# tudelft-iv/CCVPE

Hardware: AMD Instinct MI355X
Metric: image-pairs/sec (higher is better)
Workload: dtype f32

## Files before the change

ccvpe_amd/_lib.py:

```python
import ctypes
import os
import subprocess

import torch

_HERE = os.path.dirname(os.path.abspath(__file__))
LIB_PATH = os.environ.get("CCVPE_LIB") or os.path.join(_HERE, "libccvpe_hip.so")
CSRC_DIR = os.path.join(_HERE, "csrc")

c_float_p = ctypes.c_void_p
c_int = ctypes.c_int
c_float = ctypes.c_float
c_void_p = ctypes.c_void_p


class ConvDesc(ctypes.Structure):
    _fields_ = [
        ("src0", c_void_p), ("src1", c_void_p), ("gate", c_void_p), ("w", c_void_p),
        ("scale", c_void_p), ("shift", c_void_p), ("residual", c_void_p), ("dst", c_void_p),
        ("c0", c_int), ("ld0", c_int), ("c1", c_int), ("ld1", c_int),
        ("batch", c_int), ("in_h", c_int), ("in_w", c_int),
        ("kh", c_int), ("kw", c_int), ("stride", c_int), ("pad", c_int),
        ("n", c_int), ("kpad", c_int), ("ldd", c_int), ("ldres", c_int),
        ("act", c_int), ("out_mode", c_int),
# ... 6 lines not shown
        ("c0", c_int), ("ld0", c_int), ("c1", c_int), ("ld1", c_int),
        ("batch", c_int), ("h1", c_int), ("w1", c_int),
        ("n", c_int), ("kpad", c_int), ("ldd", c_int), ("act", c_int),
    ]


class TailDesc(ctypes.Structure):
    _fields_ = [
        ("x", c_void_p), ("w", c_void_p), ("shift9", c_void_p), ("w2", c_void_p), ("b2", c_void_p), ("out", c_void_p),
        ("batch", c_int), ("h1", c_int), ("w1", c_int),
        ("c0", c_int), ("ld0", c_int), ("kpad", c_int),
        ("cout", c_int), ("normalize", c_int), ("split", c_int), ("softmax_partial", c_void_p),
    ]


PROTOTYPES = {
    "ccvpe_last_error": (ctypes.c_char_p, []),
    "ccvpe_abi_version": (c_int, []),
    "ccvpe_multi_copy_f32": (c_int, [ctypes.POINTER(c_void_p), ctypes.POINTER(c_void_p), ctypes.POINTER(c_int), c_int, c_void_p]),
    "ccvpe_gather_repack_f32": (c_int, [c_void_p, c_void_p, c_void_p, c_void_p, c_void_p, c_int, c_void_p]),
    "ccvpe_gather_repack_chunk": (c_int, []),
    "ccvpe_ctx_create": (c_int, [c_void_p, ctypes.c_longlong, c_void_p, c_void_p, ctypes.POINTER(c_void_p)]),
    "ccvpe_ctx_destroy": (c_int, [c_void_p]),
    "ccvpe_ctx_info": (c_int, [c_void_p] + [ctypes.POINTER(ctypes.c_longlong)] * 4 + [ctypes.POINTER(c_int)] * 2),
    "ccvpe_ctx_output": (c_int, [c_void_p, c_int, ctypes.POINTER(c_void_p), ctypes.POINTER(ctypes.c_longlong),
                                  ctypes.POINTER(c_int), ctypes.POINTER(ctypes.c_longlong), ctypes.POINTER(ctypes.c_longlong)]),
    "ccvpe_forward": (c_int, [c_void_p, c_void_p, c_void_p, ctypes.POINTER(c_void_p), c_void_p]),
    "ccvpe_tail512_partials": (c_int, [ctypes.POINTER(TailDesc), c_int]),
    "ccvpe_softmax_apply_f32": (c_int, [c_void_p, c_void_p, c_int, c_void_p, c_int, c_int, c_void_p]),
    "ccvpe_tail512_f32": (c_int, [ctypes.POINTER(TailDesc), c_void_p]),
    "ccvpe_tail512_bf16": (c_int, [ctypes.POINTER(TailDesc), c_void_p]),
    "ccvpe_conv_igemm_f32": (c_int, [ctypes.POINTER(ConvDesc), c_void_p]),
    "ccvpe_conv_igemm_splitk_floats": (c_int, [ctypes.POINTER(ConvDesc), c_int]),
    "ccvpe_conv_igemm_route": (c_int, [ctypes.POINTER(ConvDesc), c_int, c_int]),
    "ccvpe_set_narrow_kernels": (c_int, [c_int]),
    "ccvpe_set_pw_ring_kernels": (c_int, [c_int]),
    "ccvpe_set_mbconv_plane_kernels": (c_int, [c_int]),
    "ccvpe_mbconv_front_route": (c_int, [c_int] * 8),
    "ccvpe_mbconv_band_plan": (c_int, [c_int] * 7),
    "ccvpe_conv3x3_variant": (c_int, [ctypes.POINTER(ConvDesc), c_int]),
    "ccvpe_set_match_mfma": (c_int, [c_int]),
    "ccvpe_set_pwn_kernels": (c_int, [c_int]),
    "ccvpe_conv3x3_wino_ok": (c_int, [ctypes.POINTER(ConvDesc)]),
    "ccvpe_conv3x3_wino_f32": (c_int, [ctypes.POINTER(ConvDesc), c_void_p]),
    "ccvpe_conv3x3_match1_ok": (c_int, [ctypes.POINTER(ConvDesc), c_int, c_int]),
    "ccvpe_conv3x3_match1_bf16": (c_int, [ctypes.POINTER(ConvDesc), c_int, c_void_p, c_int, c_int, c_int, c_int, c_int, c_void_p, c_void_p]),
    "ccvpe_conv_igemm_splitk_f32": (c_int, [ctypes.POINTER(ConvDesc), c_void_p, c_void_p]),
    "ccvpe_conv_igemm_splitk_bf16": (c_int, [ctypes.POINTER(ConvDesc), c_int, c_void_p, c_void_p]),
    "ccvpe_upconv3x3_f32": (c_int, [ctypes.POINTER(UpconvDesc), c_void_p]),
    "ccvpe_upconv3x3_bf16": (c_int, [ctypes.POINTER(UpconvDesc), c_void_p]),
    "ccvpe_upconv3x3_route": (c_int, [ctypes.POINTER(UpconvDesc), c_int]),
    "ccvpe_upconv3x3_s3_ok": (c_int, [ctypes.POINTER(UpconvDesc)]),
    "ccvpe_upconv3x3_s3_f32": (c_int, [ctypes.POINTER(UpconvDesc), c_void_p]),
    "ccvpe_stem_conv_f32": (c_int, [c_void_p] * 5 + [c_int] * 4 + [c_void_p]),
    "ccvpe_dwconv_nblk": (c_int, [c_int] * 4),
    "ccvpe_dwconv_f32": (c_int, [c_void_p] * 6 + [c_int] * 7 + [c_void_p]),
    "ccvpe_mbconv_front_nblk": (c_int, [c_int] * 6),
    "ccvpe_stem_dw_nblk": (c_int, [c_int] * 3),
    "ccvpe_stem_dw_f32": (c_int, [c_void_p] * 9 + [c_int] * 4 + [c_void_p]),
    "ccvpe_stem_dw_bf16": (c_int, [c_void_p] * 9 + [c_int] * 4 + [c_void_p]),
    "ccvpe_mbconv_front_f32": (c_int, [c_void_p, c_void_p, c_int] + [c_void_p] * 7 + [c_int] * 8 + [c_void_p]),
    "ccvpe_se_gate_f32": (c_int, [c_void_p, c_int, c_float] + [c_void_p] * 5 + [c_int] * 3 + [c_void_p]),
    "ccvpe_ground_descriptor_f32": (c_int, [c_void_p, c_int, c_void_p, c_void_p, ctypes.POINTER(c_int),
                                            c_void_p, c_int, c_int, c_int, c_void_p]),
    "ccvpe_match_level_f32": (c_int, [c_void_p, c_int, c_void_p, c_int, c_int, ctypes.POINTER(c_int),
                                      c_int, c_int, c_int, c_int, c_int, c_void_p, c_void_p, c_int, c_int,
                                      c_int, c_int, c_void_p]),
    "ccvpe_head_conv3x3_f32": (c_int, [c_void_p] * 4 + [c_int] * 5 + [c_void_p]),
    "ccvpe_cast_bf16_f32": (c_int, [c_void_p, c_void_p, ctypes.c_long, c_void_p]),
    "ccvpe_softmax_rows_f32": (c_int, [c_void_p, c_void_p, c_int, c_int, c_void_p]),
    "ccvpe_eval_postprocess_f32": (c_int, [c_void_p, c_void_p, c_void_p, c_int, c_int, c_int, c_void_p]),
    "ccvpe_infonce_scratch_floats": (c_int, [c_int, c_int]),
    "ccvpe_infonce_loss_f32": (c_int, [c_void_p, c_void_p, c_float, c_void_p, c_void_p, c_void_p, c_int, c_int, c_void_p]),
    "ccvpe_cross_entropy_loss_f32": (c_int, [c_void_p] * 4 + [c_int, c_int, c_void_p]),
    "ccvpe_orientation_loss_f32": (c_int, [c_void_p] * 5 + [c_int, c_int, c_void_p]),
    "ccvpe_stem_conv_raw_f32": (c_int, [c_void_p] * 3 + [c_int] * 4 + [c_void_p]),
    "ccvpe_dwconv_raw_f32": (c_int, [c_void_p] * 3 + [c_int] * 7 + [c_void_p]),
    "ccvpe_bn_stats_nblk": (c_int, [c_int]),
    "ccvpe_bn_stats_f32": (c_int, [c_void_p, c_int, c_int] + [c_void_p] * 4 + [c_float, c_void_p, c_void_p]),
    "ccvpe_bn_act_nblk": (c_int, [c_int]),
    "ccvpe_bn_act_f32": (c_int, [c_void_p] * 5 + [c_float, c_int] + [c_void_p] * 4 + [c_int] * 3 + [c_void_p]),
    "ccvpe_conv_wgrad_tile": (c_int, [c_int, c_int]),
    "ccvpe_conv_wgrad_scratch_floats": (c_int, [c_int] * 9),
    "ccvpe_conv_wgrad_f32": (c_int, [c_void_p, c_int, c_int, c_void_p, c_int, c_int, c_void_p, c_int, c_void_p,
                                     c_void_p] + [c_int] * 8 + [c_void_p]),
    "ccvpe_conv_wgrad_gated_f32": (c_int, [c_void_p, c_int, c_int, c_void_p, c_void_p, c_int, c_void_p, c_void_p, c_int, c_int, c_int,
                                           c_int, c_void_p]),
    "ccvpe_conv_wgrad_bias_f32": (c_int, [c_void_p, c_int, c_int, c_void_p, c_int, c_int, c_void_p, c_int, c_void_p,
                                          c_void_p, c_void_p] + [c_int] * 8 + [c_void_p]),
    "ccvpe_colsum_f32": (c_int, [c_void_p, c_int, c_int, c_int, c_void_p, c_void_p, c_void_p]),
    "ccvpe_bn_bwd_nblk": (c_int, [c_int]),
    "ccvpe_bn_act_bwd_f32": (c_int, [c_void_p] * 9 + [c_float, c_int] + [c_void_p] * 4 + [c_int] * 3 + [c_void_p]),
    "ccvpe_se_bn_bwd_reduce_f32": (c_int, [c_void_p] * 6 + [c_float, c_int, c_void_p, c_void_p, c_int, c_int, c_int, c_void_p]),
    "ccvpe_se_bn_bwd_apply_f32": (c_int, [c_void_p] * 8 + [c_float, c_int, c_void_p, c_void_p, c_void_p, c_void_p, c_int, c_int, c_int,
                                          c_void_p]),
    "ccvpe_se_dgate_f32": (c_int, [c_void_p] * 6 + [c_float, c_int, c_void_p] + [c_int] * 3 + [c_void_p]),
    "ccvpe_se_bwd_f32": (c_int, [c_void_p, c_int, c_float, c_void_p, c_int] + [c_void_p] * 10 + [c_int] * 3 + [c_void_p]),
    "ccvpe_dwconv_dgrad_f32": (c_int, [c_void_p] * 3 + [c_int] * 7 + [c_void_p]),
    "ccvpe_dwconv_wgrad_nblk": (c_int, [c_int] * 4),
    "ccvpe_dwconv_wgrad_f32": (c_int, [c_void_p] * 4 + [c_int] * 7 + [c_void_p]),
    "ccvpe_relu_bwd_f32": (c_int, [c_void_p] * 3 + [c_int, c_void_p]),
    "ccvpe_gate_mul_f32": (c_int, [c_void_p] * 3 + [c_int] * 3 + [c_void_p]),
    "ccvpe_softmax_bwd_f32": (c_int, [c_void_p] * 4 + [c_int, c_int, c_void_p]),
    "ccvpe_l2norm2_bwd_f32": (c_int, [c_void_p] * 3 + [c_int, c_int, c_void_p]),
    "ccvpe_head_conv3x3_bwd_f32": (c_int, [c_void_p] * 7 + [c_int] * 5 + [c_void_p]),
    "ccvpe_ground_descriptor_bwd_f32": (c_int, [c_void_p, c_int, c_void_p, ctypes.POINTER(c_int)] + [c_void_p] * 4 +
# ... 16 lines not shown
    "ccvpe_adam_step_f32": (c_int, [c_void_p, c_void_p, c_void_p, c_void_p, c_int, c_float, c_void_p]),
    "ccvpe_preprocess_u8_f32": (c_int, [c_void_p, c_int, c_int, c_void_p, c_void_p, c_int, c_void_p, c_void_p, c_int, c_void_p,
                                        c_void_p, c_int, c_int, c_int, c_int, ctypes.POINTER(c_float), ctypes.POINTER(c_float),
                                        c_void_p]),
    "ccvpe_conv_igemm_bf16": (c_int, [ctypes.POINTER(ConvDesc), c_int, c_void_p]),
    "ccvpe_stem_conv_bf16": (c_int, [c_void_p] * 5 + [c_int] * 4 + [c_void_p]),
    "ccvpe_dwconv_bf16": (c_int, [c_void_p] * 6 + [c_int] * 7 + [c_void_p]),
    "ccvpe_mbconv_front_bf16": (c_int, [c_void_p, c_void_p, c_int] + [c_void_p] * 7 + [c_int] * 8 + [c_void_p]),
    "ccvpe_match_level_bf16": (c_int, [c_void_p, c_int, c_void_p, c_int, c_int, ctypes.POINTER(c_int),
                                       c_int, c_int, c_int, c_int, c_int, c_void_p, c_void_p, c_int, c_int,
                                       c_int, c_int, c_void_p]),
    "ccvpe_head_conv3x3_bf16": (c_int, [c_void_p] * 4 + [c_int] * 5 + [c_void_p]),
}

_lib = None
weights_epoch = 0


def build(verbose=False):
    cmd = ["make", "-C", CSRC_DIR, "-j8"]
    res = subprocess.run(cmd, capture_output=True, text=True)
    if verbose or res.returncode != 0:
        print(res.stdout)
        print(res.stderr)
    if res.returncode != 0:
        raise RuntimeError("building libccvpe_hip.so failed (see output above)")
    return LIB_PATH


def load():
    global _lib
    if _lib is not None:
        return _lib
    if not os.path.isfile(LIB_PATH):
        raise RuntimeError(
            "libccvpe_hip.so not found at %s — run `python -c 'import __graft_entry__ as g; g.build()'` "
            "(or `make -C ccvpe_amd/csrc`).  ccvpe_amd has no CPU fallback." % LIB_PATH)
    lib = ctypes.CDLL(LIB_PATH)
    lax = bool(os.environ.get("CCVPE_LIB")) and os.environ.get("CCVPE_LIB_ALLOW_MISSING") == "1"
    for name, (res, args) in PROTOTYPES.items():
        if lax and not hasattr(lib, name):
            continue
        fn = getattr(lib, name)
        fn.restype = res
        fn.argtypes = args
    if os.environ.get("CCVPE_NARROW") == "0" and hasattr(lib, "ccvpe_set_narrow_kernels"):
        lib.ccvpe_set_narrow_kernels(0)
    if os.environ.get("CCVPE_PW_RING") == "0" and hasattr(lib, "ccvpe_set_pw_ring_kernels"):
        lib.ccvpe_set_pw_ring_kernels(0)
    if os.environ.get("CCVPE_MATCH_MFMA") == "0" and hasattr(lib, "ccvpe_set_match_mfma"):
        lib.ccvpe_set_match_mfma(0)
    if os.environ.get("CCVPE_PWN") == "0" and hasattr(lib, "ccvpe_set_pwn_kernels"):
        lib.ccvpe_set_pwn_kernels(0)
    if os.environ.get("CCVPE_MBPLANE") is not None and hasattr(lib, "ccvpe_set_mbconv_plane_kernels"):
        lib.ccvpe_set_mbconv_plane_kernels(int(os.environ["CCVPE_MBPLANE"]))
    _lib = lib
    return lib


class CcvpeError(RuntimeError):
    pass


def check(status, what):
    if status != 0:
        msg = load().ccvpe_last_error()
        raise CcvpeError("%s failed (%d): %s" % (what, status, msg.decode() if msg else "?"))
```

ccvpe_amd/csrc/conv_common.h:

```cpp
#pragma once
#include "common.h"
#include <cstdlib>
#include <type_traits>

namespace ccvpe {

typedef float f32x4 __attribute__((ext_vector_type(4)));
typedef __bf16 bf16_t;
typedef __bf16 bf16x8 __attribute__((ext_vector_type(8)));
typedef __bf16 bf16x4 __attribute__((ext_vector_type(4)));

template <typename T> struct ElemTraits;
template <> struct ElemTraits<float> { static constexpr int E = 4; };
template <> struct ElemTraits<bf16_t> { static constexpr int E = 8; };

template <typename T>
__device__ __forceinline__ f32x4 mfma_stage(f32x4 wfrag, f32x4 afrag, f32x4 acc);
template <>
__device__ __forceinline__ f32x4 mfma_stage<float>(f32x4 wfrag, f32x4 afrag, f32x4 acc) {
#pragma unroll
  for (int kk = 0; kk < 4; ++kk) acc = __builtin_amdgcn_mfma_f32_16x16x4f32(wfrag[kk], afrag[kk], acc, 0, 0, 0);
  return acc;
}
template <>
// ... 131 lines not shown
        else reinterpret_cast<bf16_t*>(p.dst)[obase + r] = (bf16_t)t;
      }
  }
}

#define CCVPE_ACT_DISPATCH(act, body)                                            \
  do {                                                                           \
    if ((act) == CCVPE_ACT_SWISH) body(std::integral_constant<int, CCVPE_ACT_SWISH>{});      \
    else if ((act) == CCVPE_ACT_RELU) body(std::integral_constant<int, CCVPE_ACT_RELU>{});   \
    else if ((act) == CCVPE_ACT_RELU_MASK) body(std::integral_constant<int, CCVPE_ACT_RELU_MASK>{}); \
    else body(std::integral_constant<int, CCVPE_ACT_NONE>{});                    \
  } while (0)

__device__ __forceinline__ int w_swz(int r) { return (0x1320 >> (((r >> 2) & 3) * 4)) & 3; }

struct TileCfg { int mt, nt, wn; };
static const TileCfg kCfgs[] = {
    {4, 5, 2}, {4, 4, 2}, {4, 3, 2}, {4, 2, 2}, {4, 1, 2},
    {4, 5, 1}, {4, 3, 1}, {4, 1, 1},
    {2, 7, 1},
};

static int pick_cfg(int npad16) {
  int best = 0;
  long best_cost = -1;
  for (int i = 0; i < (int)(sizeof(kCfgs) / sizeof(kCfgs[0])); ++i) {
    const int bn = 16 * kCfgs[i].nt * kCfgs[i].wn;
    const int tiles = (npad16 + bn - 1) / bn;
    const long cost = (long)tiles * bn * 1000 + (1000 - bn);
    if (best_cost < 0 || cost < best_cost) { best_cost = cost; best = i; }
  }
  return best;
}


template <typename T> int pw_dispatch(const IgemmParams& p, int mt, int nt, int wn, hipStream_t stream);
template <typename T> int conv3x3_dispatch(const IgemmParams& p, int batch, int mt, int nt, int wn, hipStream_t stream);
template <typename T> int conv3x3_variant_query(const IgemmParams& p, int batch, int mt, int nt, int wn);
extern bool g_use_pw2;
template <typename T> bool pw2_supported(const IgemmParams& p, int mt, int nt, int wn);
template <typename T> int pw2_dispatch(const IgemmParams& p, int mt, int nt, int wn, hipStream_t stream);
int num_cus();
extern bool g_use_narrow;
int c3n_supported(const IgemmParams& p, int batch);
int c3n_dispatch(const IgemmParams& p, int batch, hipStream_t stream);
int c3n_match_supported(const IgemmParams& p, int batch, int L);
int c3n_match_dispatch(const IgemmParams& p, int batch, const float* g, int ldg, int L, int off, float* scores, hipStream_t stream);
extern bool g_use_pwn;
bool pwn_supported(const IgemmParams& p, int batch, int esz);
int pwn_dispatch(const IgemmParams& p, int batch, int esz, hipStream_t stream);
int up2_supported(int c0, int c1, int n, int kpad, int h1, int w1, int batch);
int up2_dispatch(const void* src0, const void* src1, const void* w, const float* shift9, void* dst, int c0, int ld0, int c1, int ld1,
                 int h1, int w1, int n, int kpad, int ldd, int act, int batch, hipStream_t stream);

}
```

ccvpe_amd/csrc/upconv_s3.hip:

```cpp
#include "conv_common.h"

namespace ccvpe {

struct UpS3Params {
  const float* src0;
  const float* src1;
  const void* w;
  const float* shift9;
  float* dst;
  int c0, ld0, c1, ld1;
  int H1, W1, batch;
  int N, Npad;
  int nb0, nb1, nst;
  int ldd, act;
  int tiles_n, tiles_total;
};

template <int MT, int NT, int WN, bool PAIR>
struct UpS3Geom {
  static constexpr int WM = 4 / WN;
  static constexpr int BM = 16 * MT * WM;
  static constexpr int BN = 16 * NT * WN;
  static constexpr int TH = BM / 16;
  static constexpr int HR = TH + 2, HCP = PAIR ? 26 : 18;
// ... 284 lines not shown
}

template <int MT, int NT, int WN, bool PAIR>
static int launch_s3(UpS3Params p, hipStream_t stream) {
  using G = UpS3Geom<MT, NT, WN, PAIR>;
  static_assert(G::LDS_BYTES <= 80 * 1024, "upconv_s3_kernel: two workgroups per CU");
  p.tiles_n = (p.Npad + G::BN - 1) / G::BN;
  const long tiles_m = PAIR ? (p.batch + 1) / 2 : (long)((p.W1 + 15) / 16) * ((p.H1 + G::TH - 1) / G::TH) * p.batch;
  const long total = tiles_m * p.tiles_n * 4;
  if (total > 0x7fffffffL) return fail(CCVPE_EINVAL, "upconv_s3: grid too large");
  p.tiles_total = (int)total;
  static bool attr_set = false;
  if (!attr_set) {
    hipError_t e = hipFuncSetAttribute((const void*)upconv_s3_kernel<MT, NT, WN, PAIR>, hipFuncAttributeMaxDynamicSharedMemorySize, G::LDS_BYTES);
    if (e != hipSuccess) return fail(CCVPE_ELAUNCH, "upconv_s3_kernel: set smem attr: %s", hipGetErrorString(e));
    attr_set = true;
  }
  hipLaunchKernelGGL((upconv_s3_kernel<MT, NT, WN, PAIR>), dim3(p.tiles_total), dim3(256), G::LDS_BYTES, stream, p);
  return check_launch("upconv_s3_kernel");
}

static bool s3_tile(int mt, int nt, int wn) {
  return mt == 4 && ((wn == 2 && (nt == 5 || nt == 4 || nt == 2 || nt == 1)) || (wn == 1 && (nt == 5 || nt == 3)));
}

static const char* s3_refusal(const ccvpe_upconv_desc* d) {
  if (!d) return "null desc";
  if (d->c0 <= 0 || d->c0 % 8 || d->c1 <= 0 || d->c1 % 8) return "c0 / c1 must be positive multiples of 8 (a layer without a skip is not implemented)";
  if (d->batch <= 0 || d->h1 <= 0 || d->w1 <= 0 || d->n <= 0) return "bad shape";
  if (d->ld0 < d->c0 || d->ld0 % 4 || d->ld1 < d->c1 || d->ld1 % 4 || d->ldd < d->n || d->ldd % 4) return "bad strides";
  const int nst = 4 * ((d->c0 + 15) / 16) + 9 * ((d->c1 + 15) / 16);
  if (d->kpad != nst * 48) return "kpad is not that of the three-plane pack (models._pack_upconv_s3)";
  const bool pair = d->w1 == 8 && d->h1 == 8;
  if (d->w1 < 16 && !pair) return "low-res images narrower than 16 pixels (other than 8 x 8)";
  const int npad = (d->n + 15) / 16 * 16;
  const TileCfg c = kCfgs[pick_cfg(npad)];
  if (!s3_tile(c.mt, c.nt, c.wn)) return "no tile for this n";
  if (pair && !(c.nt == 5 && c.wn == 2)) return "8 x 8 images need the 160-column tile";
  const double m = (double)d->batch * d->h1 * d->w1;
  if (m * d->ld0 * 4.0 >= 4294967296.0 || 4.0 * m * d->ld1 * 4.0 >= 4294967296.0 || 4.0 * m >= 2147483648.0) return "tensor too large";
  return nullptr;
}

}

using namespace ccvpe;

extern "C" int ccvpe_upconv3x3_s3_ok(const ccvpe_upconv_desc* d) {
  if (s3_refusal(d)) return 0;
  const long m = (long)d->batch * d->h1 * d->w1;
  return m >= 4096 ? 2 : 1;
}

extern "C" int ccvpe_upconv3x3_s3_f32(const ccvpe_upconv_desc* d, void* stream) {
  if (const char* why = s3_refusal(d)) return fail(CCVPE_EINVAL, "upconv3x3_s3: %s", why);
  if (!d->src0 || !d->src1 || !d->w || !d->shift9 || !d->dst) return fail(CCVPE_EINVAL, "upconv3x3_s3: null pointer");
  if (!aligned16(d->src0) || !aligned16(d->src1) || !aligned16(d->w) || !aligned16(d->dst))
    return fail(CCVPE_EINVAL, "upconv3x3_s3: pointers must be 16-byte aligned");
  UpS3Params p;
  p.src0 = reinterpret_cast<const float*>(d->src0); p.src1 = reinterpret_cast<const float*>(d->src1);
  p.w = d->w; p.shift9 = d->shift9; p.dst = reinterpret_cast<float*>(d->dst);
  p.c0 = d->c0; p.ld0 = d->ld0; p.c1 = d->c1; p.ld1 = d->ld1;
  p.H1 = d->h1; p.W1 = d->w1; p.batch = d->batch;
  p.N = d->n; p.Npad = (d->n + 15) / 16 * 16;
  p.nb0 = (d->c0 + 15) / 16; p.nb1 = (d->c1 + 15) / 16; p.nst = 4 * p.nb0 + 9 * p.nb1;
  p.ldd = d->ldd; p.act = d->act;
  p.tiles_n = p.tiles_total = 0;
  hipStream_t st = (hipStream_t)stream;
  const TileCfg c = kCfgs[pick_cfg(p.Npad)];
  if (d->w1 == 8 && d->h1 == 8) return launch_s3<4, 5, 2, true>(p, st);
#define CCVPE_CASE(MT_, NT_, WN_) \
  if (c.mt == MT_ && c.nt == NT_ && c.wn == WN_) return launch_s3<MT_, NT_, WN_, false>(p, st);
  CCVPE_CASE(4, 5, 2) CCVPE_CASE(4, 4, 2) CCVPE_CASE(4, 2, 2) CCVPE_CASE(4, 1, 2) CCVPE_CASE(4, 5, 1) CCVPE_CASE(4, 3, 1)
#undef CCVPE_CASE
  return fail(CCVPE_EINVAL, "upconv3x3_s3: no tile config");
}
```

ccvpe_amd/ops.py:

```python
import ctypes

import torch

from . import _lib
from ._lib import ConvDesc, check

ACT_NONE, ACT_RELU, ACT_SWISH, ACT_RELU_MASK = 0, 1, 2, 3
SPLIT_K_CALLS = 0
SPLIT_K = __import__("os").environ.get("CCVPE_SPLIT_K", "1") == "1"
OUT_NHWC, OUT_DECONV2X = 0, 1

_recorder = None


def set_recorder(rec):
    global _recorder
    _recorder = rec


class LaunchRecorder(object):

    def __init__(self):
        self.items = []

# ... 230 lines not shown
    return dst


def upconv3x3(src0, c0, w_packed, shift9, n, *, batch, h1, w1, src1=None, c1=0, act=ACT_NONE, algo_flops=None, route_only=False):
    lib = _lib.load()
    dt = _act_dtype(src0)
    for t, nm in ((src0, "src0"), (src1, "src1"), (w_packed, "w")):
        _chk(t, nm, dt)
    _chk(shift9, "shift9")
    dst = _empty((batch, 2 * h1, 2 * w1, n), device=src0.device, dtype=dt)
    d = _lib.UpconvDesc()
    d.src0, d.src1, d.w, d.shift9, d.dst = _ptr(src0), _ptr(src1), _ptr(w_packed), _ptr(shift9), _ptr(dst)
    d.c0, d.ld0, d.c1, d.ld1 = c0, src0.shape[-1], c1, (src1.shape[-1] if src1 is not None else 0)
    d.batch, d.h1, d.w1 = batch, h1, w1
    d.n, d.kpad, d.ldd, d.act = n, w_packed.shape[-1], n, act
    if route_only:
        return upconv_route(d, dt != torch.float32)
    rec = _recorder
    ev0 = rec.begin() if rec is not None else None
    fn = lib.ccvpe_upconv3x3_f32 if dt == torch.float32 else lib.ccvpe_upconv3x3_bf16
    check(fn(ctypes.byref(d), _stream()), "ccvpe_upconv3x3")
    if rec is not None:
        m = batch * h1 * w1 * 4
        k_eff = 4 * c0 + 9 * c1
        flops = algo_flops if algo_flops is not None else 2.0 * m * n * k_eff
        esz = 4.0 if dt == torch.float32 else 2.0
        nbytes = esz * (batch * h1 * w1 * c0 + m * c1 + m * n + 4 * n * k_eff)
        name = upconv_route_name(d, dt != torch.float32)
        rec.end(name, "up3x3 M%d N%d Keff%d" % (m, n, k_eff), flops, nbytes, ev0)
    return dst


def _s3_desc(src0, c0, w3_packed, shift9, n, batch, h1, w1, src1, c1, act, dst, ldd, ld0, ld1):
    d = _lib.UpconvDesc()
    d.src0, d.src1, d.w, d.shift9 = _ptr(src0), _ptr(src1), _ptr(w3_packed), _ptr(shift9)
    d.dst = _ptr(dst) if dst is not None else None
    d.c0, d.ld0, d.c1, d.ld1 = c0, ld0, c1, ld1
    d.batch, d.h1, d.w1 = batch, h1, w1
    d.n, d.kpad, d.ldd, d.act = n, w3_packed.shape[1] * w3_packed.shape[3], ldd, act
    return d


def upconv3x3_s3_ok(src0, c0, w3_packed, n, *, batch, h1, w1, src1=None, c1=0, ldd=None, ld0=None, ld1=None):
    if w3_packed is None or src0.dtype != torch.float32 or (src1 is not None and src1.dtype != torch.float32):
        return 0
    if w3_packed.dtype != torch.bfloat16 or w3_packed.dim() != 4:
        return 0
    ld0 = ld0 if ld0 is not None else src0.shape[-1]
    ld1 = ld1 if ld1 is not None else (src1.shape[-1] if src1 is not None else 0)
    d = _s3_desc(src0, c0, w3_packed, None, n, batch, h1, w1, src1, c1, ACT_NONE, None, ldd if ldd is not None else n, ld0, ld1)
    return int(_lib.load().ccvpe_upconv3x3_s3_ok(ctypes.byref(d)))


def upconv3x3_s3(src0, c0, w3_packed, shift9, n, *, batch, h1, w1, src1=None, c1=0, act=ACT_NONE, dst=None, ldd=None, ld0=None,
                 ld1=None):
    lib = _lib.load()
    for t, nm in ((src0, "src0"), (src1, "src1"), (shift9, "shift9"), (dst, "dst")):
        _chk(t, nm)
    _chk(w3_packed, "w", torch.bfloat16)
    ld0 = ld0 if ld0 is not None else src0.shape[-1]
    ld1 = ld1 if ld1 is not None else (src1.shape[-1] if src1 is not None else 0)
    if dst is None:
        ldd = ldd if ldd is not None else n
        dst = _empty((batch, 2 * h1, 2 * w1, ldd), device=src0.device)
    elif ldd is None:
        ldd = dst.shape[-1]
    d = _s3_desc(src0, c0, w3_packed, shift9, n, batch, h1, w1, src1, c1, act, dst, ldd, ld0, ld1)
    rec = _recorder
    ev0 = rec.begin() if rec is not None else None
    check(lib.ccvpe_upconv3x3_s3_f32(ctypes.byref(d), _stream()), "ccvpe_upconv3x3_s3_f32")
    if rec is not None:
        m = batch * h1 * w1 * 4
        k_eff = 4 * c0 + 9 * c1
        flops = 2.0 * m * n * k_eff
        nbytes = 4.0 * (batch * h1 * w1 * c0 + m * c1 + m * n + 4 * n * k_eff)
        tile = igemm_tile(n).split("<")[1]
        name = "upconv_s3_kernel<%s%s" % (tile[:-1], ",pair>" if (h1 == 8 and w1 == 8) else ">")
        rec.end(name, "up3x3 M%d N%d Keff%d" % (m, n, k_eff), flops, nbytes, ev0)
    return dst


def tail512(x, c0, w_packed, shift9, w2, b2, cout, normalize, *, batch, h1, w1, split=False, want_softmax=False):
    lib = _lib.load()
    dt = _act_dtype(x)
    _chk(x, "x", dt)
    _chk(w_packed, "w", dt)
    for t, nm in ((shift9, "shift9"), (w2, "w2"), (b2, "b2")):
        _chk(t, nm)
    if tuple(w2.shape) != (cout, 3, 3, 16) or tuple(shift9.shape) != (9, 16) or w_packed.shape[0] != 4 or w_packed.shape[1] != 16:
        raise ValueError("tail512: w [4,16,kpad], shift9 [9,16], w2 [cout,3,3,16] expected")
    out = _empty((batch, cout, 2 * h1, 2 * w1), device=x.device, dtype=torch.float32)
    d = _lib.TailDesc()
    d.x, d.w, d.shift9, d.w2, d.b2, d.out = _ptr(x), _ptr(w_packed), _ptr(shift9), _ptr(w2), _ptr(b2), _ptr(out)
    d.batch, d.h1, d.w1 = batch, h1, w1
    d.c0, d.ld0, d.kpad = c0, x.shape[-1], w_packed.shape[-1]
    d.cout, d.normalize, d.split = cout, int(bool(normalize)), int(bool(split))
    smx = None
    if want_softmax:
        npart = lib.ccvpe_tail512_partials(ctypes.byref(d), int(dt != torch.float32))
        if npart <= 0:
            check(int(npart) if npart < 0 else -1, "ccvpe_tail512_partials")
        smx = _empty((batch, npart, 2), device=x.device, dtype=torch.float32)
        d.softmax_partial = _ptr(smx)
    rec = _recorder
    ev0 = rec.begin() if rec is not None else None
    fn = lib.ccvpe_tail512_f32 if dt == torch.float32 else lib.ccvpe_tail512_bf16
    check(fn(ctypes.byref(d), _stream()), "ccvpe_tail512")
    if rec is not None:
        m = batch * h1 * w1 * 4
        esz = 4.0 if dt == torch.float32 else 2.0
        rec.end("tail512_kernel<%s,%d>" % (("f32" if not split else "f32 as bf16 hi+lo") if dt == torch.float32 else "bf16", cout), "tail M%d Keff%d" % (m, 4 * c0),
                2.0 * m * 16 * (4 * c0 + 9 * cout), esz * batch * h1 * w1 * c0 + 4.0 * m * cout, ev0)
    return (out, smx) if want_softmax else out


def softmax_apply(logits, partials):
    lib = _lib.load()
    _chk(logits, "logits")
    _chk(partials, "partials")
    rows, n = logits.shape
    out = _empty(logits.shape, device=logits.device, dtype=logits.dtype)
    check(lib.ccvpe_softmax_apply_f32(_ptr(logits), _ptr(partials), partials.shape[1], _ptr(out), rows, n, _stream()),
          "ccvpe_softmax_apply_f32")
    return out


def tail512_ok(h1, w1, n_a):
    return n_a == 16 and h1 % 16 == 0 and w1 % 16 == 0


# ... 333 lines not shown
```

include/ccvpe_hip.h:

```cpp
#ifndef CCVPE_HIP_H
#define CCVPE_HIP_H

#ifdef __cplusplus
extern "C" {
#endif

#define CCVPE_OK 0
#define CCVPE_EINVAL (-1)
#define CCVPE_ELAUNCH (-2)

#define CCVPE_ACT_NONE 0
#define CCVPE_ACT_RELU 1
#define CCVPE_ACT_SWISH 2
#define CCVPE_ACT_RELU_MASK 3

#define CCVPE_OUT_NHWC 0
#define CCVPE_OUT_DECONV2X 1

#define CCVPE_MAX_SHIFTS 48

const char* ccvpe_last_error(void);
int ccvpe_abi_version(void);

typedef struct ccvpe_conv_desc {
// ... 9 lines not shown
  int batch, in_h, in_w;
  int kh, kw, stride, pad;
  int n;
  int kpad;
  int ldd, ldres;
  int act;
  int out_mode;
} ccvpe_conv_desc;

int ccvpe_conv_igemm_f32(const ccvpe_conv_desc* desc, void* stream);

int ccvpe_conv_igemm_splitk_floats(const ccvpe_conv_desc* desc, int is_bf16);
#define CCVPE_ROUTE_IGEMM 0
#define CCVPE_ROUTE_PW_GEMM 1
#define CCVPE_ROUTE_CONV3X3 2
#define CCVPE_ROUTE_C3N 3
#define CCVPE_ROUTE_PW_RING 4
#define CCVPE_ROUTE_PWN 5
int ccvpe_conv_igemm_route(const ccvpe_conv_desc* desc, int is_bf16, int out_f32);
int ccvpe_conv3x3_variant(const ccvpe_conv_desc* desc, int is_bf16);
int ccvpe_set_narrow_kernels(int on);
int ccvpe_set_pw_ring_kernels(int on);
int ccvpe_set_pwn_kernels(int on);
int ccvpe_set_mbconv_plane_kernels(int mode);
int ccvpe_conv3x3_wino_ok(const ccvpe_conv_desc* desc);
int ccvpe_conv3x3_wino_f32(const ccvpe_conv_desc* desc, void* stream);
int ccvpe_conv3x3_match1_ok(const ccvpe_conv_desc* desc, int out_f32, int L);
int ccvpe_conv3x3_match1_bf16(const ccvpe_conv_desc* desc, int out_f32, const float* g, int ldg, int L, int shift, int stride,
                              int window_offset, float* scores, void* stream);
int ccvpe_conv_igemm_splitk_f32(const ccvpe_conv_desc* desc, float* scratch, void* stream);

typedef struct ccvpe_upconv_desc {
  const void* src0;
  const void* src1;
  const void* w;
  const float* shift9;
  void* dst;
  int c0, ld0, c1, ld1;
  int batch, h1, w1;
  int n, kpad, ldd;
  int act;
} ccvpe_upconv_desc;

int ccvpe_upconv3x3_f32(const ccvpe_upconv_desc* desc, void* stream);
int ccvpe_upconv3x3_bf16(const ccvpe_upconv_desc* desc, void* stream);
#define CCVPE_UPROUTE_GATHER 0
#define CCVPE_UPROUTE_HALO 1
#define CCVPE_UPROUTE_DMA 2
#define CCVPE_UPROUTE_DMA_PAIR 3
#define CCVPE_UPROUTE_UP2 4
int ccvpe_upconv3x3_route(const ccvpe_upconv_desc* desc, int is_bf16);
int ccvpe_upconv3x3_s3_ok(const ccvpe_upconv_desc* desc);
int ccvpe_upconv3x3_s3_f32(const ccvpe_upconv_desc* desc, void* stream);

typedef struct ccvpe_tail_desc {
  const void* x;
  const void* w;
  const float* shift9;
  const float* w2;
  const float* b2;
  float* out;
  int batch, h1, w1;
  int c0, ld0, kpad;
  int cout, normalize, split;
  float* softmax_partial;
} ccvpe_tail_desc;

int ccvpe_tail512_f32(const ccvpe_tail_desc* desc, void* stream);
int ccvpe_tail512_bf16(const ccvpe_tail_desc* desc, void* stream);
int ccvpe_tail512_partials(const ccvpe_tail_desc* desc, int is_bf16);
int ccvpe_softmax_apply_f32(const float* logits, const float* partials, int n_partials, float* out, int rows, int n,
                            void* stream);

typedef struct ccvpe_ctx ccvpe_ctx;
int ccvpe_ctx_create(const void* plan, long long n_bytes, void* weights_dev, void* workspace_dev, ccvpe_ctx** ctx);
int ccvpe_ctx_destroy(ccvpe_ctx* ctx);
int ccvpe_ctx_info(const ccvpe_ctx* ctx, long long* workspace_bytes, long long* weights_bytes, long long* grd_bytes,
                   long long* sat_bytes, int* n_outputs, int* n_calls);
int ccvpe_ctx_output(const ccvpe_ctx* ctx, int i, void** dev_ptr, long long* bytes, int* ndim, long long* dims4,
                     long long* strides4);
int ccvpe_forward(ccvpe_ctx* ctx, const void* grd, const void* sat, void** out, void* stream);

int ccvpe_stem_conv_f32(const float* x_nchw, const float* w, const float* scale, const float* shift,
                        float* y, int batch, int in_h, int in_w, int circular, void* stream);

int ccvpe_dwconv_nblk(int in_h, int in_w, int channels, int stride);
int ccvpe_dwconv_f32(const float* x, const float* w, const float* scale, const float* shift, float* y,
                     float* se_partial, int batch, int in_h, int in_w, int channels, int k, int stride,
                     int circular, void* stream);

int ccvpe_stem_dw_nblk(int in_h, int in_w, int circular);
int ccvpe_stem_dw_f32(const float* x_nchw, const float* w, const float* s0, const float* b0, const float* w_dw,
                      const float* s1, const float* b1, float* y, float* se_partial, int batch, int in_h,
                      int in_w, int circular, void* stream);
int ccvpe_stem_dw_bf16(const float* x_nchw, const float* w, const float* s0, const float* b0, const float* w_dw,
                       const float* s1, const float* b1, void* y, float* se_partial, int batch, int in_h,
                       int in_w, int circular, void* stream);

int ccvpe_mbconv_front_nblk(int in_h, int in_w, int cin, int mid, int k, int stride);
int ccvpe_mbconv_front_route(int in_h, int in_w, int cin, int mid, int k, int stride, int is_bf16, int batch);
int ccvpe_mbconv_band_plan(int in_h, int in_w, int cin, int mid, int k, int stride, int batch);
int ccvpe_mbconv_front_f32(const float* x, const float* w_exp, int kpad, const float* s0, const float* b0,
                           const float* w_dw, const float* s1, const float* b1, float* y, float* se_partial,
                           int batch, int in_h, int in_w, int cin, int mid, int k, int stride, int circular,
                           void* stream);

// ... 153 lines not shown
```

Baseline: 2602.

## Add quad-parity upconv s3 kernel that computes all four output parities per tile

Adds a new upconv3x3 s3 kernel that accumulates all four output parities of the 2x deconvolution in one workgroup. The upsampled skip input is staged once into parity-split LDS planes as three-way bf16 splits of f32, and weights are fed by DMA double-buffering. This replaces separate per-parity passes, cutting repeated halo and skip-input loads and launches. It is auto-selected for 16<n<=80, row width >=16 and M>=4096, with an env switch to disable it. The cost is a heavy LDS footprint and more MFMA work from the split-precision emulation.

New measurement: 2665, median of 6. 2.4% higher.

```diff
diff --git a/ccvpe_amd/_lib.py b/ccvpe_amd/_lib.py
--- a/ccvpe_amd/_lib.py
+++ b/ccvpe_amd/_lib.py
@@ -82,6 +82,9 @@
     "ccvpe_upconv3x3_route": (c_int, [ctypes.POINTER(UpconvDesc), c_int]),
     "ccvpe_upconv3x3_s3_ok": (c_int, [ctypes.POINTER(UpconvDesc)]),
     "ccvpe_upconv3x3_s3_f32": (c_int, [ctypes.POINTER(UpconvDesc), c_void_p]),
+    "ccvpe_upconv3x3_s3_form_ok": (c_int, [ctypes.POINTER(UpconvDesc), c_int]),
+    "ccvpe_upconv3x3_s3_form_f32": (c_int, [ctypes.POINTER(UpconvDesc), c_int, c_void_p]),
+    "ccvpe_set_s3_quad": (c_int, [c_int]),
     "ccvpe_stem_conv_f32": (c_int, [c_void_p] * 5 + [c_int] * 4 + [c_void_p]),
     "ccvpe_dwconv_nblk": (c_int, [c_int] * 4),
     "ccvpe_dwconv_f32": (c_int, [c_void_p] * 6 + [c_int] * 7 + [c_void_p]),
@@ -204,6 +207,8 @@
         lib.ccvpe_set_match_mfma(0)
     if os.environ.get("CCVPE_PWN") == "0" and hasattr(lib, "ccvpe_set_pwn_kernels"):
         lib.ccvpe_set_pwn_kernels(0)
+    if os.environ.get("CCVPE_S3_QUAD") == "0" and hasattr(lib, "ccvpe_set_s3_quad"):
+        lib.ccvpe_set_s3_quad(0)
     if os.environ.get("CCVPE_MBPLANE") is not None and hasattr(lib, "ccvpe_set_mbconv_plane_kernels"):
         lib.ccvpe_set_mbconv_plane_kernels(int(os.environ["CCVPE_MBPLANE"]))
     _lib = lib
diff --git a/ccvpe_amd/csrc/conv_common.h b/ccvpe_amd/csrc/conv_common.h
--- a/ccvpe_amd/csrc/conv_common.h
+++ b/ccvpe_amd/csrc/conv_common.h
@@ -207,5 +207,7 @@
 int up2_supported(int c0, int c1, int n, int kpad, int h1, int w1, int batch);
 int up2_dispatch(const void* src0, const void* src1, const void* w, const float* shift9, void* dst, int c0, int ld0, int c1, int ld1,
                  int h1, int w1, int n, int kpad, int ldd, int act, int batch, hipStream_t stream);
-
-}
+bool upconv_s3q_serves(const ccvpe_upconv_desc* d);
+int upconv_s3q_launch(const ccvpe_upconv_desc* d, hipStream_t stream);
+
+}
diff --git a/ccvpe_amd/csrc/upconv_s3.hip b/ccvpe_amd/csrc/upconv_s3.hip
--- a/ccvpe_amd/csrc/upconv_s3.hip
+++ b/ccvpe_amd/csrc/upconv_s3.hip
@@ -360,11 +360,35 @@
   return m >= 4096 ? 2 : 1;
 }
 
-extern "C" int ccvpe_upconv3x3_s3_f32(const ccvpe_upconv_desc* d, void* stream) {
+static bool g_s3_quad = true;
+static int s3_auto_form(const ccvpe_upconv_desc* d) {
+  if (!g_s3_quad || !upconv_s3q_serves(d)) return 1;
+  const long m = (long)d->batch * d->h1 * d->w1;
+  return m >= 4096 ? 2 : 1;
+}
+
+extern "C" int ccvpe_set_s3_quad(int on) {
+  const int prev = g_s3_quad ? 1 : 0;
+  g_s3_quad = on != 0;
+  return prev;
+}
+
+extern "C" int ccvpe_upconv3x3_s3_form_ok(const ccvpe_upconv_desc* d, int form) {
+  if (s3_refusal(d)) return 0;
+  if (form == 0) return s3_auto_form(d);
+  if (form == 1) return 1;
+  if (form == 2) return upconv_s3q_serves(d) ? 2 : 0;
+  return 0;
+}
+
+static int s3_run(const ccvpe_upconv_desc* d, int form, void* stream) {
   if (const char* why = s3_refusal(d)) return fail(CCVPE_EINVAL, "upconv3x3_s3: %s", why);
+  if (form < 0 || form > 2) return fail(CCVPE_EINVAL, "upconv3x3_s3: form must be 0 (auto), 1 (per-parity) or 2 (quad)");
   if (!d->src0 || !d->src1 || !d->w || !d->shift9 || !d->dst) return fail(CCVPE_EINVAL, "upconv3x3_s3: null pointer");
   if (!aligned16(d->src0) || !aligned16(d->src1) || !aligned16(d->w) || !aligned16(d->dst))
     return fail(CCVPE_EINVAL, "upconv3x3_s3: pointers must be 16-byte aligned");
+  if (form == 0) form = s3_auto_form(d);
+  if (form == 2) return upconv_s3q_launch(d, (hipStream_t)stream);
   UpS3Params p;
   p.src0 = reinterpret_cast<const float*>(d->src0); p.src1 = reinterpret_cast<const float*>(d->src1);
   p.w = d->w; p.shift9 = d->shift9; p.dst = reinterpret_cast<float*>(d->dst);
@@ -383,3 +407,7 @@
 #undef CCVPE_CASE
   return fail(CCVPE_EINVAL, "upconv3x3_s3: no tile config");
 }
+
+extern "C" int ccvpe_upconv3x3_s3_f32(const ccvpe_upconv_desc* d, void* stream) { return s3_run(d, 0, stream); }
+
+extern "C" int ccvpe_upconv3x3_s3_form_f32(const ccvpe_upconv_desc* d, int form, void* stream) { return s3_run(d, form, stream); }
diff --git a/ccvpe_amd/csrc/upconv_s3q.hip b/ccvpe_amd/csrc/upconv_s3q.hip
--- /dev/null
+++ b/ccvpe_amd/csrc/upconv_s3q.hip
@@ -0,0 +1,348 @@
+#include "conv_common.h"
+
+namespace ccvpe {
+
+struct UpS3qParams {
+  const float* src0;
+  const float* src1;
+  const void* w;
+  const float* shift9;
+  float* dst;
+  int c0, ld0, c1, ld1;
+  int H1, W1, batch;
+  int N;
+  int nb0, nb1, nst;
+  int ldd, act;
+  int tiles_total;
+};
+
+template <int NT>
+struct UpS3qGeom {
+  static constexpr int TH = 8, HR = TH + 2, HC = 18;
+  static constexpr int PR = TH + 1, PC = 17;
+  static constexpr int ROW = 24;
+  static constexpr int NP = 16 * NT;
+  static constexpr int HALO_DW = HR * HC * ROW;
+  static constexpr int PLANES_DW = 4 * PR * PC * ROW;
+  static constexpr int WA_INSTR = 6 * NT;
+  static constexpr int WA_DW = WA_INSTR * 256;
+  static constexpr int WB_INSTR = (NP * 6 + 63) / 64;
+  static constexpr int WB_DW = WB_INSTR * 256;
+  static constexpr int G = NT == 2 ? 3 : (NT == 3 ? 2 : 1);
+  static constexpr int A_DW = HALO_DW + 2 * WA_DW;
+  static constexpr int B_DW = PLANES_DW + 2 * G * WB_DW;
+  static constexpr int LDS_BYTES = (A_DW > B_DW ? A_DW : B_DW) * 4;
+};
+
+__device__ __forceinline__ unsigned q_pk_bf16(float a, float b) {
+  typedef __bf16 bf16x2_t __attribute__((ext_vector_type(2)));
+  bf16x2_t v;
+  v[0] = (__bf16)a;
+  v[1] = (__bf16)b;
+  return __builtin_bit_cast(unsigned, v);
+}
+__device__ __forceinline__ float q_bf_lo(unsigned p) { return __builtin_bit_cast(float, p << 16); }
+__device__ __forceinline__ float q_bf_hi(unsigned p) { return __builtin_bit_cast(float, p & 0xffff0000u); }
+
+typedef unsigned q_u32x2 __attribute__((ext_vector_type(2)));
+__device__ __forceinline__ void q_store_planes(float* at, f32x4 v) {
+  q_u32x2 hi, mid, lo;
+#pragma unroll
+  for (int h = 0; h < 2; ++h) {
+    float a = v[2 * h], b = v[2 * h + 1];
+    const unsigned ph = q_pk_bf16(a, b);
+    a -= q_bf_lo(ph);
+    b -= q_bf_hi(ph);
+    const unsigned pm = q_pk_bf16(a, b);
+    a -= q_bf_lo(pm);
+    b -= q_bf_hi(pm);
+    hi[h] = ph;
+    mid[h] = pm;
+    lo[h] = q_pk_bf16(a, b);
+  }
+  *reinterpret_cast<q_u32x2*>(at) = hi;
+  *reinterpret_cast<q_u32x2*>(at + 8) = mid;
+  *reinterpret_cast<q_u32x2*>(at + 16) = lo;
+}
+
+template <int NT>
+__global__ __launch_bounds__(256, 2) void upconv_s3q_kernel(const UpS3qParams p) {
+  using G = UpS3qGeom<NT>;
+  constexpr int TH = G::TH, HR = G::HR, HC = G::HC, PR = G::PR, PC = G::PC, ROW = G::ROW, NP = G::NP;
+  constexpr int HPX = HR * HC;
+  constexpr int H_IT = (HPX * 4 + 255) / 256;
+  constexpr int SPX = (2 * TH + 2) * 34;
+  constexpr int S_IT = 5, S_HALVES = (SPX * 4 + 256 * S_IT - 1) / (256 * S_IT);
+  constexpr int NGRP = 36 / G::G;
+
+  extern __shared__ __attribute__((aligned(16))) float s3q_sm[];
+  float* Us = s3q_sm;
+  float* WsA = s3q_sm + G::HALO_DW;
+  float* WsB = s3q_sm + G::PLANES_DW;
+
+  const int tid = threadIdx.x;
+  const int lane = tid & 63;
+  const int wave = sgpr(tid >> 6);
+
+  const int tile = xcd_tile(blockIdx.x, p.tiles_total);
+  const int tiles_x = (p.W1 + 15) / 16;
+  const int tiles_y = (p.H1 + TH - 1) / TH;
+  const int tx = tile % tiles_x;
+  const int ty = (tile / tiles_x) % tiles_y;
+  const int b = tile / (tiles_x * tiles_y);
+  const int y0 = ty * TH, x0 = tx * 16;
+  const int H2 = 2 * p.H1, W2 = 2 * p.W1;
+  const int ld0s = sgpr(p.ld0), ld1s = sgpr(p.ld1);
+
+  int h_off[H_IT], h_pix[H_IT], h_sub[H_IT];
+#pragma unroll
+  for (int it = 0; it < H_IT; ++it) {
+    const int idx = tid + 256 * it;
+    const int pxl = idx >> 2, sub = idx & 3;
+    h_sub[it] = sub;
+    if (pxl < HPX) {
+      const int hy = pxl / HC, hx = pxl - hy * HC;
+      const int iy = y0 - 1 + hy, ix = x0 - 1 + hx;
+      h_off[it] = (hy * HC + hx) * ROW + sub * 2;
+      h_pix[it] = ((unsigned)iy < (unsigned)p.H1 && (unsigned)ix < (unsigned)p.W1) ? (b * p.H1 + iy) * p.W1 + ix : -1;
+    } else {
+      h_off[it] = -1;
+      h_pix[it] = -1;
+    }
+  }
+  f32x4 h_reg[H_IT];
+  unsigned h_keep = 0;
+  auto load_halo = [&](int chunk) {
+    h_keep = 0;
+#pragma unroll
+    for (int it = 0; it < H_IT; ++it) {
+      const int ch = chunk * 16 + h_sub[it] * 4;
+      const bool ok = h_pix[it] >= 0 && ch < p.c0;
+      h_reg[it] = *reinterpret_cast<const f32x4*>(reinterpret_cast<const char*>(p.src0) + (ok ? ((unsigned)h_pix[it] * (unsigned)ld0s + (unsigned)ch) * 4u : 0u));
+      h_keep |= ok ? (1u << it) : 0u;
+    }
+  };
+  auto store_halo = [&]() {
+#pragma unroll
+    for (int it = 0; it < H_IT; ++it)
+      if (h_off[it] >= 0) q_store_planes(Us + h_off[it], keep_if(h_reg[it], (h_keep >> it) & 1u));
+  };
+
+  auto stage_planes = [&](int blk) {
+#pragma unroll
+    for (int half = 0; half < S_HALVES; ++half) {
+      f32x4 r[S_IT];
+      int off[S_IT];
+      unsigned keep = 0;
+#pragma unroll
+      for (int it = 0; it < S_IT; ++it) {
+        const int idx = tid + 256 * (half * S_IT + it);
+        const int pxl = idx >> 2, sub = idx & 3;
+        const int hy = pxl / 34, hx = pxl - hy * 34;
+        const int iy = 2 * y0 - 1 + hy, ix = 2 * x0 - 1 + hx;
+        const int ch = blk * 16 + sub * 4;
+        const bool ok = pxl < SPX && (unsigned)iy < (unsigned)H2 && (unsigned)ix < (unsigned)W2 && ch < p.c1;
+        const unsigned goff = ok ? ((unsigned)((b * H2 + iy) * W2 + ix) * (unsigned)ld1s + (unsigned)ch) * 4u : 0u;
+        r[it] = *reinterpret_cast<const f32x4*>(reinterpret_cast<const char*>(p.src1) + goff);
+        keep |= ok ? (1u << it) : 0u;
+        off[it] = pxl < SPX ? ((((hy & 1) * 2 + (hx & 1)) * PR + (hy >> 1)) * PC + (hx >> 1)) * ROW + sub * 2 : -1;
+      }
+#pragma unroll
+      for (int it = 0; it < S_IT; ++it)
+        if (off[it] >= 0) q_store_planes(Us + off[it], keep_if(r[it], (keep >> it) & 1u));
+    }
+  };
+
+  const unsigned lds0 = (unsigned)(uintptr_t)(__attribute__((address_space(3))) float*)s3q_sm;
+  const unsigned vlin = (unsigned)lane * 16u;
+  const unsigned vlast = (unsigned)min(lane, 31) * 16u;
+  const size_t stage_bytes = (size_t)NP * (ROW * 4);
+  auto dma_one = [&](unsigned lds, unsigned voff, const char* sbase) {
+    const unsigned l = __builtin_amdgcn_readfirstlane(lds);
+    asm volatile("s_mov_b32 m0, %0\n\tglobal_load_lds_dwordx4 %1, %2" ::"s"(l), "v"(voff), "s"(sbase) : "memory", "m0");
+  };
+  auto dma_a = [&](int chunk, int par, int buf) {
+    const char* sbase = reinterpret_cast<const char*>(p.w) + ((size_t)par * p.nst + (size_t)chunk * 4) * stage_bytes;
+#pragma unroll
+    for (int q = 0; q < (G::WA_INSTR + 3) / 4; ++q) {
+      const int g = wave + 4 * q;
+      if (g < G::WA_INSTR) dma_one(lds0 + (unsigned)((G::HALO_DW + buf * G::WA_DW + g * 256) * 4), vlin, sbase + (size_t)g * 1024);
+    }
+  };
+  auto dma_b = [&](int blk, int grp) {
+#pragma unroll
+    for (int q = 0; q < (G::G * G::WB_INSTR + 3) / 4; ++q) {
+      const int e = wave + 4 * q;
+      if (e < G::G * G::WB_INSTR) {
+        const int u = e / G::WB_INSTR, g = e - u * G::WB_INSTR;
+        const int seq = grp * G::G + u;
+        const int par = seq / 9, tap = seq - 9 * par;
+        const char* sbase = reinterpret_cast<const char*>(p.w) + ((size_t)par * p.nst + (size_t)(4 * p.nb0 + tap * p.nb1 + blk)) * stage_bytes + (size_t)g * 1024;
+        const bool half = (NT & 1) && g == G::WB_INSTR - 1;
+        dma_one(lds0 + (unsigned)((G::PLANES_DW + ((grp & 1) * G::G + u) * G::WB_DW + g * 256) * 4), half ? vlast : vlin, sbase);
+      }
+    }
+  };
+  auto dma_wait = [&]() { asm volatile("s_waitcnt vmcnt(0)" ::: "memory"); };
+
+  f32x4 acc[4][2][NT];
+#pragma unroll
+  for (int q = 0; q < 4; ++q)
+#pragma unroll
+    for (int i = 0; i < 2; ++i)
+#pragma unroll
+      for (int j = 0; j < NT; ++j) acc[q][i][j] = (f32x4){0.f, 0.f, 0.f, 0.f};
+  const int frow = lane & 15;
+  const int g4 = lane >> 4;
+  const int a1off = 4 * g4;
+  const int a2off = g4 < 2 ? 16 + 4 * g4 : 4 * g4 - 8;
+  const int w1off = 4 * (g4 & 1);
+  const int w2off = 8 + 4 * (g4 & 1);
+  const int w3off = g4 < 2 ? 4 * g4 : 4 * g4 + 8;
+
+#define CCVPE_S3Q_TAP(PAR, abase, istride, wb)                                                              \
+  {                                                                                                         \
+    f32x4 a1[2], a2[2];                                                                                     \
+    _Pragma("unroll") for (int i = 0; i < 2; ++i) {                                                         \
+      a1[i] = *reinterpret_cast<const f32x4*>((abase) + i * (istride) + a1off);                             \
+      a2[i] = *reinterpret_cast<const f32x4*>((abase) + i * (istride) + a2off);                             \
+    }                                                                                                       \
+    _Pragma("unroll") for (int j = 0; j < NT; ++j) {                                                        \
+      const f32x4 w1 = *reinterpret_cast<const f32x4*>((wb) + j * 16 * ROW + w1off);                        \
+      const f32x4 w2 = *reinterpret_cast<const f32x4*>((wb) + j * 16 * ROW + w2off);                        \
+      const f32x4 w3 = *reinterpret_cast<const f32x4*>((wb) + j * 16 * ROW + w3off);                        \
+      _Pragma("unroll") for (int i = 0; i < 2; ++i) acc[PAR][i][j] = mfma_stage<bf16_t>(w1, a1[i], acc[PAR][i][j]); \
+      _Pragma("unroll") for (int i = 0; i < 2; ++i) acc[PAR][i][j] = mfma_stage<bf16_t>(w2, a1[i], acc[PAR][i][j]); \
+      _Pragma("unroll") for (int i = 0; i < 2; ++i) acc[PAR][i][j] = mfma_stage<bf16_t>(w3, a2[i], acc[PAR][i][j]); \
+    }                                                                                                       \
+  }
+
+  const float* hfrag = Us + (wave * 2 * HC + frow) * ROW;
+  const float* wfrag_a = WsA + frow * ROW;
+  load_halo(0);
+  dma_a(0, 0, 0);
+  store_halo();
+  dma_wait();
+  __syncthreads();
+  for (int chunk = 0; chunk < p.nb0; ++chunk) {
+    const bool next_halo = chunk + 1 < p.nb0;
+    if (next_halo) load_halo(chunk + 1);
+#pragma unroll
+    for (int par = 0; par < 4; ++par) {
+      if (par < 3) dma_a(chunk, par + 1, (par + 1) & 1);
+      else if (next_halo) dma_a(chunk + 1, 0, 0);
+      const int py = par >> 1, px = par & 1;
+#pragma unroll
+      for (int tap = 0; tap < 4; ++tap) {
+        const int du = tap >> 1, dv = tap & 1;
+        CCVPE_S3Q_TAP(par, hfrag + ((du + py) * HC + dv + px) * ROW, HC * ROW, wfrag_a + ((par & 1) * G::WA_DW + tap * NP * ROW));
+      }
+      dma_wait();
+      __syncthreads();
+    }
+    if (next_halo) {
+      store_halo();
+      __syncthreads();
+    }
+  }
+
+  const float* pfrag = Us + (wave * 2 * PC + frow) * ROW;
+  const float* wfrag_b = WsB + frow * ROW;
+  for (int blk = 0; blk < p.nb1; ++blk) {
+    dma_b(blk, 0);
+    stage_planes(blk);
+    dma_wait();
+    __syncthreads();
+#pragma unroll
+    for (int grp = 0; grp < NGRP; ++grp) {
+      if (grp + 1 < NGRP) dma_b(blk, grp + 1);
+#pragma unroll
+      for (int u = 0; u < G::G; ++u) {
+        const int seq = grp * G::G + u;
+        const int par = seq / 9, tap = seq % 9;
+        const int r = (par >> 1) + tap / 3, c = (par & 1) + tap % 3;
+        CCVPE_S3Q_TAP(par, pfrag + ((((r & 1) * 2 + (c & 1)) * PR + (r >> 1)) * PC + (c >> 1)) * ROW, PC * ROW,
+                      wfrag_b + ((grp & 1) * G::G + u) * G::WB_DW);
+      }
+      dma_wait();
+      __syncthreads();
+    }
+  }
+#undef CCVPE_S3Q_TAP
+
+  const int epix = lane & 15;
+  const int en = (lane >> 4) * 4;
+  IgemmParams ep{};
+  ep.N = p.N; ep.act = p.act; ep.residual = nullptr; ep.dst = p.dst; ep.out_f32 = 1;
+  const float one[4] = {1.f, 1.f, 1.f, 1.f};
+  const int x1 = x0 + epix;
+  auto epilogue = [&](auto act_tag) {
+  constexpr int ACT = decltype(act_tag)::value;
+#pragma unroll
+  for (int par = 0; par < 4; ++par) {
+    const int py = par >> 1, px = par & 1;
+#pragma unroll
+    for (int i = 0; i < 2; ++i) {
+      const int y1 = y0 + wave * 2 + i;
+      if (y1 >= p.H1 || x1 >= p.W1) continue;
+      const int Y = 2 * y1 + py, X = 2 * x1 + px;
+      const int rc = Y == 0 ? 0 : (Y == H2 - 1 ? 2 : 1);
+      const int cc = X == 0 ? 0 : (X == W2 - 1 ? 2 : 1);
+      const float* shp = p.shift9 + (size_t)(rc * 3 + cc) * p.N;
+      const size_t pix = (size_t)(b * H2 + Y) * W2 + X;
+#pragma unroll
+      for (int j = 0; j < NT; ++j) {
+        const int n = j * 16 + en;
+        if (n >= p.N) continue;
+        float sh[4];
+#pragma unroll
+        for (int q = 0; q < 4; ++q) sh[q] = (n + q < p.N) ? shp[n + q] : 0.f;
+        store4<float, ACT>(ep, acc[par][i][j], n, pix * p.ldd + n, 0, one, sh);
+      }
+    }
+  }
+  };
+  CCVPE_ACT_DISPATCH(p.act, epilogue);
+}
+
+template <int NT>
+static int launch_s3q(UpS3qParams p, hipStream_t stream) {
+  using G = UpS3qGeom<NT>;
+  static_assert(G::LDS_BYTES <= 80 * 1024, "upconv_s3q_kernel: two workgroups per CU");
+  p.tiles_total = ((p.W1 + 15) / 16) * ((p.H1 + G::TH - 1) / G::TH) * p.batch;
+  static bool attr_set = false;
+  if (!attr_set) {
+    hipError_t e = hipFuncSetAttribute((const void*)upconv_s3q_kernel<NT>, hipFuncAttributeMaxDynamicSharedMemorySize, G::LDS_BYTES);
+    if (e != hipSuccess) return fail(CCVPE_ELAUNCH, "upconv_s3q_kernel: set smem attr: %s", hipGetErrorString(e));
+    attr_set = true;
+  }
+  hipLaunchKernelGGL((upconv_s3q_kernel<NT>), dim3(p.tiles_total), dim3(256), G::LDS_BYTES, stream, p);
+  return check_launch("upconv_s3q_kernel");
+}
+
+bool upconv_s3q_serves(const ccvpe_upconv_desc* d) {
+  const int npad = (d->n + 15) / 16 * 16;
+  return d->w1 >= 16 && npad >= 32 && npad <= 80;
+}
+
+int upconv_s3q_launch(const ccvpe_upconv_desc* d, hipStream_t stream) {
+  if (!upconv_s3q_serves(d)) return fail(CCVPE_EINVAL, "upconv3x3_s3: the quad form serves 16 < n <= 80 and images of 16 or more pixels a row");
+  UpS3qParams p;
+  p.src0 = reinterpret_cast<const float*>(d->src0); p.src1 = reinterpret_cast<const float*>(d->src1);
+  p.w = d->w; p.shift9 = d->shift9; p.dst = reinterpret_cast<float*>(d->dst);
+  p.c0 = d->c0; p.ld0 = d->ld0; p.c1 = d->c1; p.ld1 = d->ld1;
+  p.H1 = d->h1; p.W1 = d->w1; p.batch = d->batch;
+  p.N = d->n;
+  p.nb0 = (d->c0 + 15) / 16; p.nb1 = (d->c1 + 15) / 16; p.nst = 4 * p.nb0 + 9 * p.nb1;
+  p.ldd = d->ldd; p.act = d->act;
+  p.tiles_total = 0;
+  switch ((d->n + 15) / 16) {
+    case 2: return launch_s3q<2>(p, stream);
+    case 3: return launch_s3q<3>(p, stream);
+    case 4: return launch_s3q<4>(p, stream);
+    case 5: return launch_s3q<5>(p, stream);
+  }
+  return fail(CCVPE_EINVAL, "upconv3x3_s3: no quad tile");
+}
+
+}
diff --git a/ccvpe_amd/ops.py b/ccvpe_amd/ops.py
--- a/ccvpe_amd/ops.py
+++ b/ccvpe_amd/ops.py
@@ -306,8 +306,17 @@
     return int(_lib.load().ccvpe_upconv3x3_s3_ok(ctypes.byref(d)))
 
 
+def upconv3x3_s3_form_ok(src0, c0, w3_packed, n, form, *, batch, h1, w1, src1=None, c1=0, ldd=None, ld0=None, ld1=None):
+    if not upconv3x3_s3_ok(src0, c0, w3_packed, n, batch=batch, h1=h1, w1=w1, src1=src1, c1=c1, ldd=ldd, ld0=ld0, ld1=ld1):
+        return 0
+    ld0 = ld0 if ld0 is not None else src0.shape[-1]
+    ld1 = ld1 if ld1 is not None else (src1.shape[-1] if src1 is not None else 0)
+    d = _s3_desc(src0, c0, w3_packed, None, n, batch, h1, w1, src1, c1, ACT_NONE, None, ldd if ldd is not None else n, ld0, ld1)
+    return int(_lib.load().ccvpe_upconv3x3_s3_form_ok(ctypes.byref(d), form))
+
+
 def upconv3x3_s3(src0, c0, w3_packed, shift9, n, *, batch, h1, w1, src1=None, c1=0, act=ACT_NONE, dst=None, ldd=None, ld0=None,
-                 ld1=None):
+                 ld1=None, form=None):
     lib = _lib.load()
     for t, nm in ((src0, "src0"), (src1, "src1"), (shift9, "shift9"), (dst, "dst")):
         _chk(t, nm)
@@ -322,7 +331,10 @@
     d = _s3_desc(src0, c0, w3_packed, shift9, n, batch, h1, w1, src1, c1, act, dst, ldd, ld0, ld1)
     rec = _recorder
     ev0 = rec.begin() if rec is not None else None
-    check(lib.ccvpe_upconv3x3_s3_f32(ctypes.byref(d), _stream()), "ccvpe_upconv3x3_s3_f32")
+    if form is None:
+        check(lib.ccvpe_upconv3x3_s3_f32(ctypes.byref(d), _stream()), "ccvpe_upconv3x3_s3_f32")
+    else:
+        check(lib.ccvpe_upconv3x3_s3_form_f32(ctypes.byref(d), form, _stream()), "ccvpe_upconv3x3_s3_form_f32")
     if rec is not None:
         m = batch * h1 * w1 * 4
         k_eff = 4 * c0 + 9 * c1
@@ -330,6 +342,8 @@
         nbytes = 4.0 * (batch * h1 * w1 * c0 + m * c1 + m * n + 4 * n * k_eff)
         tile = igemm_tile(n).split("<")[1]
         name = "upconv_s3_kernel<%s%s" % (tile[:-1], ",pair>" if (h1 == 8 and w1 == 8) else ">")
+        if lib.ccvpe_upconv3x3_s3_form_ok(ctypes.byref(d), form or 0) == 2:
+            name = "upconv_s3q_kernel<2,%d>" % ((n + 15) // 16)
         rec.end(name, "up3x3 M%d N%d Keff%d" % (m, n, k_eff), flops, nbytes, ev0)
     return dst
 
diff --git a/include/ccvpe_hip.h b/include/ccvpe_hip.h
--- a/include/ccvpe_hip.h
+++ b/include/ccvpe_hip.h
@@ -85,6 +85,9 @@
 int ccvpe_upconv3x3_route(const ccvpe_upconv_desc* desc, int is_bf16);
 int ccvpe_upconv3x3_s3_ok(const ccvpe_upconv_desc* desc);
 int ccvpe_upconv3x3_s3_f32(const ccvpe_upconv_desc* desc, void* stream);
+int ccvpe_upconv3x3_s3_form_ok(const ccvpe_upconv_desc* desc, int form);
+int ccvpe_upconv3x3_s3_form_f32(const ccvpe_upconv_desc* desc, int form, void* stream);
+int ccvpe_set_s3_quad(int on);
 
 typedef struct ccvpe_tail_desc {
   const void* x;
```
